# samuel-watson/glmmrMCML

Measured on AMD Instinct MI355X. Metric: MCML iters/sec x m chains (simlik evals/sec), higher is better.
Workload: dtype f64

## Files before the change

### glmmrmcml_amd/csrc/debug_hooks.hip

```cpp
#include "dgemm_mfma.h"
#include "dgemm_dl.h"
#include "dgemm_band.h"

using namespace mcml;

extern "C" int glmmr_mcml_dbg_dgemm(int M, int N, int K, const double* A, int lda,
                                    const double* B, int ldb, int b_nmajor,
                                    double alpha, double beta, double* C, int ldc,
                                    int lower_only, int force_tile)
{
    int ndev = 0;
    if (hipGetDeviceCount(&ndev) != hipSuccess || ndev == 0) {
        set_error("no HIP device: libglmmr_mcml_hip has no CPU fallback");
        return MCML_ENODEVICE;
    }
    hipStream_t s = nullptr;
    DevMat dA, dB, dC;
    if (force_tile == 40) {
        MCML_REQUIRE(!b_nmajor && !lower_only, "dbg_dgemm: the direct-to-LDS kernel takes a K-major B and all tiles");
        const int kpad = round_up(K, 32);
        MCML_TRY(dA.alloc(M, K, 32));
        MCML_HIP(hipMemset(dA.d(), 0, sizeof(double) * (size_t)dA.ld * dA.cols_alloc));
        MCML_HIP(hipMemcpy2D(dA.d(), sizeof(double) * dA.ld, A, sizeof(double) * lda, sizeof(double) * M, K, hipMemcpyHostToDevice));
        MCML_TRY(dB.alloc(kpad, N));
        MCML_HIP(hipMemset(dB.d(), 0, sizeof(double) * (size_t)dB.ld * N));
        MCML_HIP(hipMemcpy2D(dB.d(), sizeof(double) * dB.ld, B, sizeof(double) * ldb, sizeof(double) * K, N, hipMemcpyHostToDevice));
        MCML_TRY(upload_matrix(dC, C, M, N, ldc, s));
        MCML_REQUIRE(dlds_applicable(M, N, K, dA.d(), dA.ld, dA.cols_alloc, dB.d(), dB.ld), "dbg_dgemm: operands do not meet the direct-to-LDS contract");
        EpiAxpby epi2{dC.d(), dC.ld, alpha, beta};
        MCML_TRY(launch_gemm_dlds(s, M, N, K, dA.d(), dA.ld, dB.d(), dB.ld, epi2));
        MCML_TRY(download_matrix(C, ldc, dC.d(), dC.ld, M, N, s));
        return MCML_OK;
    }
    MCML_TRY(upload_matrix(dA, A, M, K, lda, s));
    if (b_nmajor) MCML_TRY(upload_matrix(dB, B, N, K, ldb, s));
    else MCML_TRY(upload_matrix(dB, B, K, N, ldb, s));
    MCML_TRY(upload_matrix(dC, C, M, N, ldc, s));
    EpiAxpby epi{dC.d(), dC.ld, alpha, beta};
    int rc;
    if (force_tile >= 20)
        rc = b_nmajor ? launch_gemm_dl<true>(s, M, N, K, dA.d(), dA.ld, dB.d(), dB.ld, epi, lower_only != 0, force_tile - 19)
                      : launch_gemm_dl<false>(s, M, N, K, dA.d(), dA.ld, dB.d(), dB.ld, epi, lower_only != 0, force_tile - 19);
    else
        rc = b_nmajor ? launch_gemm<true>(s, M, N, K, dA.d(), dA.ld, dB.d(), dB.ld, epi, lower_only != 0, force_tile)
                      : launch_gemm<false>(s, M, N, K, dA.d(), dA.ld, dB.d(), dB.ld, epi, lower_only != 0, force_tile);
    MCML_TRY(rc);
    MCML_TRY(download_matrix(C, ldc, dC.d(), dC.ld, M, N, s));
    return MCML_OK;
}

extern "C" int glmmr_mcml_dbg_dgemm_bench2(int M, int N, int K, int b_nmajor, int iters, int force_tile,
                                           int lower_only, double beta, double* ms_per_launch);
extern "C" int glmmr_mcml_dbg_dgemm_bench(int M, int N, int K, int b_nmajor, int iters,
                                          int force_tile, double* ms_per_launch)
{
    return glmmr_mcml_dbg_dgemm_bench2(M, N, K, b_nmajor, iters, force_tile, 0, 0.0, ms_per_launch);
}

extern "C" int glmmr_mcml_dbg_dgemm_bench2(int M, int N, int K, int b_nmajor, int iters, int force_tile,
                                           int lower_only, double beta, double* ms_per_launch)
{
    int ndev = 0;
    if (hipGetDeviceCount(&ndev) != hipSuccess || ndev == 0) {
        set_error("no HIP device: libglmmr_mcml_hip has no CPU fallback");
        return MCML_ENODEVICE;
    }
    hipStream_t s = nullptr;
    std::vector<double> hA((size_t)M * K), hB((size_t)K * N), hC((size_t)M * N, 0.0);
    uint64_t x = 88172645463325252ULL;
    auto rnd = [&]() { x ^= x << 13; x ^= x >> 7; x ^= x << 17; return (double)(x >> 11) / 9007199254740992.0 * 2 - 1; };
    for (auto& v : hA) v = rnd();
    for (auto& v : hB) v = rnd();
    DevMat dA, dB, dC;
    MCML_TRY(upload_matrix(dA, hA.data(), M, K, M, s));
    if (b_nmajor) MCML_TRY(upload_matrix(dB, hB.data(), N, K, N, s));
    else MCML_TRY(upload_matrix(dB, hB.data(), K, N, K, s));
    MCML_TRY(upload_matrix(dC, hC.data(), M, N, M, s));
    EpiAxpby epi{dC.d(), dC.ld, beta != 0.0 ? 1e-3 : 1.0, beta};
    const bool lo = lower_only != 0;
    auto go = [&]() {
        if (force_tile >= 20)
            return b_nmajor ? launch_gemm_dl<true>(s, M, N, K, dA.d(), dA.ld, dB.d(), dB.ld, epi, lo, force_tile - 19)
                            : launch_gemm_dl<false>(s, M, N, K, dA.d(), dA.ld, dB.d(), dB.ld, epi, lo, force_tile - 19);
        return b_nmajor ? launch_gemm<true>(s, M, N, K, dA.d(), dA.ld, dB.d(), dB.ld, epi, lo, force_tile)
                        : launch_gemm<false>(s, M, N, K, dA.d(), dA.ld, dB.d(), dB.ld, epi, lo, force_tile);
    };
    for (int i = 0; i < 3; i++) MCML_TRY(go());
    hipEvent_t e0, e1;
    MCML_HIP(hipEventCreate(&e0));
    MCML_HIP(hipEventCreate(&e1));
    MCML_HIP(hipEventRecord(e0, s));
    for (int i = 0; i < iters; i++) MCML_TRY(go());
    MCML_HIP(hipEventRecord(e1, s));
    MCML_HIP(hipEventSynchronize(e1));
    float ms = 0;
    MCML_HIP(hipEventElapsedTime(&ms, e0, e1));
    *ms_per_launch = ms / iters;
    (void)hipEventDestroy(e0);
    (void)hipEventDestroy(e1);
    return MCML_OK;
}

extern "C" int glmmr_mcml_dbg_dgemm_band(int M, int N, int K, const double* A, int lda, const double* B, int ldb,
                                         double* C, int ldc, int* tiles_executed)
{
    int ndev = 0;
    if (hipGetDeviceCount(&ndev) != hipSuccess || ndev == 0) {
        set_error("no HIP device: libglmmr_mcml_hip has no CPU fallback");
        return MCML_ENODEVICE;
    }
    MCML_REQUIRE(M > 0 && N > 0 && K > 0 && A && B && C, "dbg_dgemm_band: bad argument");
    hipStream_t s = nullptr;
    DevMat dA, dB, dC;
    MCML_TRY(dA.alloc(M, K, 32));
    MCML_HIP(hipMemset(dA.d(), 0, sizeof(double) * (size_t)dA.ld * dA.cols_alloc));
    MCML_HIP(hipMemcpy2D(dA.d(), sizeof(double) * dA.ld, A, sizeof(double) * lda, sizeof(double) * M, K, hipMemcpyHostToDevice));
    MCML_TRY(dB.alloc(round_up(K, 32), N));
    MCML_HIP(hipMemset(dB.d(), 0, sizeof(double) * (size_t)dB.ld * N));
    MCML_HIP(hipMemcpy2D(dB.d(), sizeof(double) * dB.ld, B, sizeof(double) * ldb, sizeof(double) * K, N, hipMemcpyHostToDevice));
    MCML_TRY(dC.alloc(M, N));
    MCML_HIP(hipMemset(dC.d(), 0, sizeof(double) * (size_t)dC.ld * N));
    MCML_REQUIRE(dlds_applicable(M, N, K, dA.d(), dA.ld, dA.cols_alloc, dB.d(), dB.ld), "dbg_dgemm_band: contract");
    const int nbands = (M + BD_BM - 1) / BD_BM;
    DevBuf kr;
    MCML_TRY(kr.ensure(sizeof(int) * 2 * nbands));
    hipLaunchKernelGGL(k_band_ranges, dim3(nbands), dim3(256), 0, s, dA.d(), dA.ld, M, K, kr.as<int>());
    MCML_HIP(hipGetLastError());
    std::vector<int> hk(2 * nbands);
    MCML_HIP(hipMemcpy(hk.data(), kr.p, sizeof(int) * 2 * nbands, hipMemcpyDeviceToHost));
    BandPlan plan;
    plan.reset(M, K, hk);
    if (tiles_executed) *tiles_executed = (int)plan.tiles;
    EpiAxpby epi{dC.d(), dC.ld, 1.0, 0.0};
    MCML_TRY(launch_gemm_band(s, plan, N, dA.d(), dA.ld, dB.d(), dB.ld, epi));
    MCML_TRY(download_matrix(C, ldc, dC.d(), dC.ld, M, N, s));
    return MCML_OK;
}

extern "C" int glmmr_mcml_dbg_band_clocks(int M, int N, int iters, int mode, double* out3)
{
    int ndev = 0;
    if (hipGetDeviceCount(&ndev) != hipSuccess || ndev == 0) {
        set_error("no HIP device: libglmmr_mcml_hip has no CPU fallback");
        return MCML_ENODEVICE;
    }
    hipStream_t s = nullptr;
    if (getenv("GLMMR_MCML_DBG_STREAM")) MCML_HIP(hipStreamCreateWithFlags(&s, hipStreamNonBlocking));
    std::vector<double> hA((size_t)M * M, 0.0), hB((size_t)M * N);
    uint64_t x = 88172645463325252ULL;
    auto rnd = [&]() { x ^= x << 13; x ^= x >> 7; x ^= x << 17; return (double)(x >> 11) / 9007199254740992.0 * 2 - 1; };
    const bool cst = getenv("GLMMR_MCML_DBG_DATA") && !strcmp(getenv("GLMMR_MCML_DBG_DATA"), "const");
    const bool dec = getenv("GLMMR_MCML_DBG_DATA") && !strcmp(getenv("GLMMR_MCML_DBG_DATA"), "decay");
    for (int j = 0; j < M; ++j) for (int i = j; i < M; ++i) hA[i + (size_t)j * M] = cst ? 1.0 : dec ? rnd() * std::exp(-(double)(i - j) / 40.0) : rnd();
    for (auto& v : hB) v = cst ? 1.0 : rnd();
    DevMat dA, dB, dC;
    MCML_TRY(dA.alloc(M, M, 32));
    MCML_HIP(hipMemset(dA.d(), 0, sizeof(double) * (size_t)dA.ld * dA.cols_alloc));
    MCML_HIP(hipMemcpy2D(dA.d(), sizeof(double) * dA.ld, hA.data(), sizeof(double) * M, sizeof(double) * M, M, hipMemcpyHostToDevice));
    MCML_TRY(dB.alloc(round_up(M, 32), N));
    MCML_HIP(hipMemset(dB.d(), 0, sizeof(double) * (size_t)dB.ld * N));
    MCML_HIP(hipMemcpy2D(dB.d(), sizeof(double) * dB.ld, hB.data(), sizeof(double) * M, sizeof(double) * M, N, hipMemcpyHostToDevice));
    MCML_TRY(dC.alloc(M, N));
    const int nbands = (M + BD_BM - 1) / BD_BM;
    DevBuf kr, clk;
    MCML_TRY(kr.ensure(sizeof(int) * 2 * nbands));
    MCML_TRY(clk.ensure(16));
    MCML_HIP(hipMemset(clk.p, 0, 16));
    hipLaunchKernelGGL(k_band_ranges, dim3(nbands), dim3(256), 0, s, dA.d(), dA.ld, M, M, kr.as<int>());
    std::vector<int> hk(2 * nbands);
    MCML_HIP(hipMemcpy(hk.data(), kr.p, sizeof(int) * 2 * nbands, hipMemcpyDeviceToHost));
    BandPlan plan;
    plan.reset(M, M, hk);
    const double tiles = (double)plan.tiles;
    EpiAxpby epi{dC.d(), dC.ld, 1.0, 0.0};
    if (mode < 0) {
        for (int i = 0; i < 3; i++)
            MCML_TRY((launch_gemm_band<EpiAxpby, false>(s, plan, N, dA.d(), dA.ld, dB.d(), dB.ld, epi)));
        hipEvent_t f0, f1;
        MCML_HIP(hipEventCreate(&f0));
        MCML_HIP(hipEventCreate(&f1));
        MCML_HIP(hipEventRecord(f0, s));
        for (int i = 0; i < iters; i++)
            MCML_TRY((launch_gemm_band<EpiAxpby, false>(s, plan, N, dA.d(), dA.ld, dB.d(), dB.ld, epi)));
        MCML_HIP(hipEventRecord(f1, s));
        MCML_HIP(hipEventSynchronize(f1));
        float fms = 0;
        MCML_HIP(hipEventElapsedTime(&fms, f0, f1));
        out3[0] = fms / iters; out3[1] = 0;
        out3[2] = 2.0 * 80.0 * 32.0 * tiles * N / (fms / iters * 1e-3) / 1e12;
        (void)hipEventDestroy(f0);
        (void)hipEventDestroy(f1);
        return MCML_OK;
    }
    if (mode & 16) {
        BandPlanDev* d = nullptr;
        MCML_TRY(plan.device_plan((N + BD_BN - 1) / BD_BN, s, &d));
        const int nb = d->nwg * d->gn;
        DevBuf st;
        MCML_TRY(st.ensure(sizeof(unsigned long long) * (8 + 8 * (size_t)nb)));
        for (int rep = 0; rep < 3; ++rep) {
            MCML_HIP(hipMemset(st.p, 0, sizeof(unsigned long long) * (8 + 8 * (size_t)nb)));
            MCML_TRY((launch_gemm_band<EpiAxpby, true>(s, plan, N, dA.d(), dA.ld, dB.d(), dB.ld, epi, st.as<unsigned long long>(), mode)));
            MCML_HIP(hipDeviceSynchronize());
        }
        std::vector<unsigned long long> h(8 + 8 * (size_t)nb);
        MCML_HIP(hipMemcpy(h.data(), st.p, sizeof(unsigned long long) * h.size(), hipMemcpyDeviceToHost));
        unsigned long long t0 = ~0ULL;
        for (int w = 0; w < nb; ++w) if (h[8 + 8 * w] && h[8 + 8 * w] < t0) t0 = h[8 + 8 * w];
        double mx[5] = {0, 0, 0, 0, 0}, sm[5] = {0, 0, 0, 0, 0};
        for (int w = 0; w < nb; ++w)
            for (int i = 0; i < 5; ++i) { double v = (double)(h[8 + 8 * w + i] - t0) * 0.01; sm[i] += v; if (v > mx[i]) mx[i] = v; }
        printf("band stamps (us from the first workgroup's start; %d workgroups, mean / max):\n", nb);
        const char* nm[5] = {"start", "ring filled", "K loop done", "epilogue issued", "end"};
        for (int i = 0; i < 5; ++i) printf("  %-16s %7.2f / %7.2f\n", nm[i], sm[i] / nb, mx[i]);
        if (mode & 32) for (int w = 0; w < nb; ++w) {
            printf("  wg %3d:", w);
            for (int i = 0; i < 5; ++i) printf(" %7.2f", (double)(h[8 + 8 * w + i] - t0) * 0.01);
            printf("\n");
        }
        fflush(stdout);
        out3[0] = out3[1] = out3[2] = 0;
        return MCML_OK;
    }
    for (int i = 0; i < 3; i++)
        MCML_TRY((launch_gemm_band<EpiAxpby, true>(s, plan, N, dA.d(), dA.ld, dB.d(), dB.ld, epi)));
    hipEvent_t e0, e1;
    MCML_HIP(hipEventCreate(&e0));
    MCML_HIP(hipEventCreate(&e1));
    MCML_HIP(hipEventRecord(e0, s));
    for (int i = 0; i < iters; i++)
        MCML_TRY((launch_gemm_band<EpiAxpby, true>(s, plan, N, dA.d(), dA.ld, dB.d(), dB.ld, epi, clk.as<unsigned long long>(), mode)));
    MCML_HIP(hipEventRecord(e1, s));
    MCML_HIP(hipEventSynchronize(e1));
    float ms = 0;
    MCML_HIP(hipEventElapsedTime(&ms, e0, e1));
    unsigned long long hc[2] = {0, 0};
    MCML_HIP(hipMemcpy(hc, clk.p, 16, hipMemcpyDeviceToHost));
    out3[0] = ms / iters;
    out3[1] = hc[1] ? (double)hc[0] / (double)hc[1] * 100.0 : 0.0;
    out3[2] = 2.0 * 80.0 * 32.0 * tiles * N / (ms / iters * 1e-3) / 1e12;
    (void)hipEventDestroy(e0);
    (void)hipEventDestroy(e1);
    return MCML_OK;
}

extern "C" const char* glmmr_mcml_last_error(void) { return mcml::last_error(); }

#include "rng.h"
__global__ void k_dbg_normals(uint64_t seed, uint32_t chain, uint32_t prop, uint32_t tag, int n, double* out)
{
    int i = blockIdx.x * blockDim.x + threadIdx.x;
    if (i < n) out[i] = rng_normal(seed, (uint32_t)i, chain, prop, tag);
}
__global__ void k_dbg_minstd(uint32_t seed, int n, double* out)
{
    if (threadIdx.x || blockIdx.x) return;
    uint32_t x = seed % 2147483647u;
    if (x == 0) x = 1;
    for (int i = 0; i < n; ++i) out[i] = minstd_canonical(x);
}
extern "C" int glmmr_mcml_dbg_normals(uint64_t seed, uint32_t chain, uint32_t prop, uint32_t tag, int n,
                                      double* out)
{
    DevBuf b;
    MCML_TRY(b.ensure(sizeof(double) * (size_t)n));
    hipLaunchKernelGGL(k_dbg_normals, dim3((n + 255) / 256), dim3(256), 0, nullptr, seed, chain, prop, tag, n, b.d());
    MCML_HIP(hipGetLastError());
    MCML_HIP(hipMemcpy(out, b.p, sizeof(double) * (size_t)n, hipMemcpyDeviceToHost));
    return MCML_OK;
}
extern "C" int glmmr_mcml_dbg_minstd(uint32_t seed, int n, double* out)
{
    DevBuf b;
    MCML_TRY(b.ensure(sizeof(double) * (size_t)n));
    hipLaunchKernelGGL(k_dbg_minstd, dim3(1), dim3(64), 0, nullptr, seed, n, b.d());
    MCML_HIP(hipGetLastError());
    MCML_HIP(hipMemcpy(out, b.p, sizeof(double) * (size_t)n, hipMemcpyDeviceToHost));
    return MCML_OK;
}

#include "../../include/glmmr_mcml_c.h"
#include "optim.h"
#include <cmath>
extern "C" int glmmr_mcml_dbg_bobyqa(glmmr_mcml_objective f, void* user, int n, const double* x0,
                                     const double* lower, const double* upper, double rhobeg, double rhoend,
                                     int maxfun, double* x_out, double* f_out, int* nfev_out)
{
    MCML_REQUIRE(f && n > 0 && x0 && x_out, "dbg_bobyqa: bad argument");
    objective_fn obj = [&](const std::vector<double>& x, double* v) { *v = f(x.data(), n, user); return 0; };
    std::vector<double> x(x0, x0 + n), lo(n, -HUGE_VAL), up(n, HUGE_VAL);
    if (lower) lo.assign(lower, lower + n);
    if (upper) up.assign(upper, upper + n);
    BobyqaOpts o; o.rhobeg = rhobeg; o.rhoend = rhoend; if (maxfun > 0) o.maxfun = maxfun;
    BobyqaResult r;
    MCML_TRY(bobyqa(obj, x, lo, up, o, &r));
    for (int i = 0; i < n; ++i) x_out[i] = r.x[i];
    if (f_out) *f_out = r.fval;
    if (nfev_out) *nfev_out = r.nfev;
    return MCML_OK;
}
extern "C" int glmmr_mcml_dbg_bobyqa_batch(glmmr_mcml_objective f, void* user, int n, const double* x0,
                                           const double* lower, const double* upper, double rhobeg, double rhoend,
                                           int maxfun, int width, double* x_out, double* f_out, int* nfev_out,
                                           int* rounds_out)
{
    MCML_REQUIRE(f && n > 0 && x0 && x_out && width >= 1, "dbg_bobyqa_batch: bad argument");
    batch_objective_fn obj = [&](const std::vector<std::vector<double>>& X, std::vector<double>* F) {
        F->resize(X.size());
        for (size_t i = 0; i < X.size(); ++i) (*F)[i] = f(X[i].data(), n, user);
        return 0; };
    std::vector<double> x(x0, x0 + n), lo(n, -HUGE_VAL), up(n, HUGE_VAL);
    if (lower) lo.assign(lower, lower + n);
    if (upper) up.assign(upper, upper + n);
    BobyqaOpts o; o.rhobeg = rhobeg; o.rhoend = rhoend; if (maxfun > 0) o.maxfun = maxfun;
    BobyqaResult r;
    MCML_TRY(bobyqa_batch(obj, x, lo, up, o, width, &r));
    for (int i = 0; i < n; ++i) x_out[i] = r.x[i];
    if (f_out) *f_out = r.fval;
    if (nfev_out) *nfev_out = r.nfev;
    if (rounds_out) *rounds_out = r.rounds;
    return MCML_OK;
}
extern "C" int glmmr_mcml_dbg_bobyqa_rounds(glmmr_mcml_batch_objective fb, void* user, int n, const double* x0,
                                            const double* lower, const double* upper, double rhobeg, double rhoend,
                                            int maxfun, int width, double* x_out, double* f_out, int* nfev_out,
                                            int* rounds_out)
{
    MCML_REQUIRE(fb && n > 0 && x0 && x_out && width >= 1, "dbg_bobyqa_rounds: bad argument");
    batch_objective_fn obj = [&](const std::vector<std::vector<double>>& X, std::vector<double>* F) {
        const int k = (int)X.size();
        std::vector<double> flat((size_t)n * k);
        for (int j = 0; j < k; ++j) for (int i = 0; i < n; ++i) flat[(size_t)j * n + i] = X[j][i];
        F->assign(k, 0.0);
        return fb(flat.data(), n, k, F->data(), user); };
    std::vector<double> x(x0, x0 + n), lo(n, -HUGE_VAL), up(n, HUGE_VAL);
    if (lower) lo.assign(lower, lower + n);
    if (upper) up.assign(upper, upper + n);
    BobyqaOpts o; o.rhobeg = rhobeg; o.rhoend = rhoend; if (maxfun > 0) o.maxfun = maxfun;
    BobyqaResult r;
    MCML_TRY(bobyqa_batch(obj, x, lo, up, o, width, &r));
    for (int i = 0; i < n; ++i) x_out[i] = r.x[i];
    if (f_out) *f_out = r.fval;
    if (nfev_out) *nfev_out = r.nfev;
    if (rounds_out) *rounds_out = r.rounds;
    return MCML_OK;
}
extern "C" int glmmr_mcml_dbg_fd_hessian(glmmr_mcml_objective f, void* user, int n, const double* x, double ndeps,
                                         int usebounds, const double* lower, const double* upper, double* H)
{
    MCML_REQUIRE(f && n > 0 && x && H, "dbg_fd_hessian: bad argument");
    objective_fn obj = [&](const std::vector<double>& xx, double* v) { *v = f(xx.data(), n, user); return 0; };
    std::vector<double> xv(x, x + n), nd(n, ndeps), lo(n, -HUGE_VAL), up(n, HUGE_VAL), h;
    if (lower) lo.assign(lower, lower + n);
    if (upper) up.assign(upper, upper + n);
    MCML_TRY(fd_hessian(obj, xv, nd, usebounds != 0, lo, up, &h));
    for (int i = 0; i < n * n; ++i) H[i] = h[i];
    return MCML_OK;
}

extern "C" int glmmr_mcml_dbg_copy_roundtrip(const double* in, long long ld_in, double* out, long long ld_out, long long rows, long long cols)
{
    MCML_REQUIRE(in && out && rows > 0 && cols > 0 && ld_in >= rows && ld_out >= rows, "copy_roundtrip: bad arguments");
    const size_t ldd = (size_t)rows + 3;
    DevBuf buf;
    MCML_TRY(buf.ensure(sizeof(double) * ldd * (size_t)cols));
    MCML_HIP(hipMemset(buf.p, 0xff, sizeof(double) * ldd * (size_t)cols));
    MCML_TRY(copy_h2d_2d(buf.p, sizeof(double) * ldd, in, sizeof(double) * (size_t)ld_in, sizeof(double) * (size_t)rows, (size_t)cols, 0));
    MCML_TRY(copy_d2h_2d(out, sizeof(double) * (size_t)ld_out, buf.p, sizeof(double) * ldd, sizeof(double) * (size_t)rows, (size_t)cols, 0));
    MCML_HIP(hipDeviceSynchronize());
    return MCML_OK;
}
```

### glmmrmcml_amd/csrc/dgemm_dl.h

```cpp
#pragma once
#include "dgemm_dlds.h"

namespace mcml {

template <int WTM, int WTN, int WM, int WN, bool BNMAJOR, int STAGES>
struct DlgCfg {
    static constexpr int BK = 16;
    static constexpr int NW = WM * WN, THREADS = 64 * NW;
    static constexpr int BM = 16 * WTM * WM, BN = 16 * WTN * WN;
    static constexpr int A_BYTES = BK * BM * 8, B_BYTES = BK * BN * 8;
    static constexpr int A_CHUNKS = A_BYTES / 1024, B_CHUNKS = B_BYTES / 1024;
    static constexpr int CHUNKS = A_CHUNKS + B_CHUNKS;
    static constexpr int PER = (CHUNKS + NW - 1) / NW;
    static constexpr int STAGE_BYTES = A_BYTES + B_BYTES;
    static constexpr size_t LDS_BYTES = (size_t)STAGES * STAGE_BYTES;
    static constexpr bool SWZ_A = (BM % 32) == 0;
    static constexpr bool SWZ_B = BNMAJOR && (BN % 32) == 0;
    static_assert(BM % 8 == 0 && BN % 8 == 0, "tile sides are multiples of 8 doubles");
    static_assert(LDS_BYTES <= 160 * 1024, "LDS ring does not fit");
    static_assert(PER * (STAGES - 1) <= 24, "vmcnt immediates in dl_wait_vm");
};

template <int N>
__device__ __forceinline__ void dl_wait_vm()
{
#define MCML_VM(n) else if constexpr (N == n) asm volatile("s_waitcnt vmcnt(" #n ")" ::: "memory");
    if constexpr (N <= 0) asm volatile("s_waitcnt vmcnt(0)" ::: "memory");
    MCML_VM(1) MCML_VM(2) MCML_VM(3) MCML_VM(4) MCML_VM(5) MCML_VM(6) MCML_VM(7) MCML_VM(8)
    MCML_VM(9) MCML_VM(10) MCML_VM(11) MCML_VM(12) MCML_VM(13) MCML_VM(14) MCML_VM(15) MCML_VM(16)
    MCML_VM(17) MCML_VM(18) MCML_VM(19) MCML_VM(20) MCML_VM(21) MCML_VM(22) MCML_VM(23) MCML_VM(24)
    else asm volatile("s_waitcnt vmcnt(0)" ::: "memory");
#undef MCML_VM
}

template <int PER, int MAXT>
__device__ __forceinline__ void dl_wait_leave(int tiles)
{
    if constexpr (MAXT <= 0) dl_wait_vm<0>();
    else {
        if (tiles >= MAXT) dl_wait_vm<PER * MAXT>();
        else dl_wait_leave<PER, MAXT - 1>(tiles);
    }
}

template <int WTM, int WTN, int WM, int WN, bool BNMAJOR, int STAGES, class Epi>
__global__ __launch_bounds__(64 * WM * WN) void dgemm_dl_kernel(GemmP p, Epi epi)
{
    using Cfg = DlgCfg<WTM, WTN, WM, WN, BNMAJOR, STAGES>;
    constexpr int BM = Cfg::BM, BN = Cfg::BN, BK = Cfg::BK, NW = Cfg::NW, PER = Cfg::PER;
    extern __shared__ __attribute__((aligned(16))) double smem[];
    char* lds = reinterpret_cast<char*>(smem);
    const int tid = threadIdx.x, lane = tid & 63, wave = __builtin_amdgcn_readfirstlane(tid >> 6);
    const int wr = wave / WN, wc = wave - wr * WN;

    const int nblk = gridDim.x;
    const int bid = blockIdx.x;
    const int q8 = nblk >> 3, r8 = nblk & 7, xcd = bid & 7;
    const int nid = (xcd < r8 ? xcd * (q8 + 1) : r8 * (q8 + 1) + (xcd - r8) * q8) + (bid >> 3);
    int bi, bj;
    if (p.lower_only) {
        int rem = nid;
        for (bi = 0; bi < p.gm; ++bi) {
            int nc = (bi * BM + BM - 1 + p.diag_shift) / BN + 1;
            if (nc > p.gn) nc = p.gn;
            if (rem < nc) break;
            rem -= nc;
        }
        bj = rem;
    } else {
        bi = nid / p.gn; bj = nid - bi * p.gn;
    }
    const int m0 = bi * BM, n0 = bj * BN;

    unsigned voff[PER]; int loff[PER]; bool isA[PER];
#pragma unroll
    for (int s = 0; s < PER; ++s) {
        int c = wave + NW * s;
        if (c >= Cfg::CHUNKS) c = wave;
        isA[s] = c < Cfg::A_CHUNKS;
        if (c < Cfg::A_CHUNKS) {
            const int o = c * 1024 + lane * 16;
            const int k = o / (BM * 8), pos = (o - k * BM * 8) >> 3;
            const int m = Cfg::SWZ_A ? ((((pos >> 4) ^ (k & 1)) << 4) | (pos & 15)) : pos;
            int gm = m0 + m;
            if (gm >= p.M) gm = 0;
            voff[s] = (unsigned)((gm + (size_t)k * p.lda) * 8);
            loff[s] = c * 1024;
        } else {
            const int cb = c - Cfg::A_CHUNKS;
            const int o = cb * 1024 + lane * 16;
            if (BNMAJOR) {
                const int k = o / (BN * 8), pos = (o - k * BN * 8) >> 3;
                const int n = Cfg::SWZ_B ? ((((pos >> 4) ^ (k & 1)) << 4) | (pos & 15)) : pos;
                int gn = n0 + n;
                if (gn >= p.N) gn = 0;
                voff[s] = (unsigned)((gn + (size_t)k * p.ldb) * 8);
            } else {
                const int q = o >> 4;
                const int kp = q / BN, n = q - kp * BN;
                int gn = n0 + n;
                if (gn >= p.N) gn = 0;
                voff[s] = (unsigned)((2 * kp + (size_t)gn * p.ldb) * 8);
            }
            loff[s] = Cfg::A_BYTES + cb * 1024;
        }
    }
    const size_t stepA = (size_t)BK * p.lda * 8, stepB = BNMAJOR ? (size_t)BK * p.ldb * 8 : (size_t)BK * 8;
    const int by = blockIdx.y;
    const char* sA = reinterpret_cast<const char*>(p.A + (size_t)by * p.bsA);
    const char* sB = reinterpret_cast<const char*>(p.B + (size_t)by * p.bsB);

    auto issue = [&](int stage) {
        const unsigned lbase = (unsigned)(size_t)(lds_ptr_t)lds + stage * Cfg::STAGE_BYTES;
#pragma unroll
        for (int s = 0; s < PER; ++s) lds_dma16(lbase + loff[s], voff[s], isA[s] ? sA : sB);
        sA += stepA;
        sB += stepB;
    };

    d4 acc[WTM][WTN];
#pragma unroll
    for (int i = 0; i < WTM; ++i)
#pragma unroll
        for (int j = 0; j < WTN; ++j) acc[i][j] = d4{0.0, 0.0, 0.0, 0.0};

    const int l15 = lane & 15, lk = lane >> 4;
    auto compute = [&](int stage) {
        const double* as = reinterpret_cast<const double*>(lds + stage * Cfg::STAGE_BYTES);
        const double* bs = reinterpret_cast<const double*>(lds + stage * Cfg::STAGE_BYTES + Cfg::A_BYTES);
#pragma unroll
        for (int ks = 0; ks < BK / 4; ++ks) {
            const int kk = 4 * ks + lk;
            double a[WTM], b[WTN];
#pragma unroll
            for (int i = 0; i < WTM; ++i) {
                const int blk = wr * WTM + i;
                a[i] = as[kk * BM + ((Cfg::SWZ_A ? (blk ^ (kk & 1)) : blk) << 4) + l15];
            }
#pragma unroll
            for (int j = 0; j < WTN; ++j) {
                const int blk = wc * WTN + j;
                if (BNMAJOR) b[j] = bs[kk * BN + ((Cfg::SWZ_B ? (blk ^ (kk & 1)) : blk) << 4) + l15];
                else b[j] = bs[((kk >> 1) * BN + (blk << 4) + l15) * 2 + (kk & 1)];
            }
#pragma unroll
            for (int i = 0; i < WTM; ++i)
#pragma unroll
                for (int j = 0; j < WTN; ++j)
                    acc[i][j] = __builtin_amdgcn_mfma_f64_16x16x4f64(b[j], a[i], acc[i][j], 0, 0, 0);
        }
    };

    const int nk = p.K / BK;
    int issued = 0;
    for (; issued < STAGES - 1 && issued < nk; ++issued) issue(issued);
    dl_wait_leave<PER, STAGES - 2>(issued - 1);
    __builtin_amdgcn_s_barrier();
    int st = 0;
    for (int kt = 0; kt < nk; ++kt) {
        if (issued < nk) {
            int sn = st + STAGES - 1; if (sn >= STAGES) sn -= STAGES;
            issue(sn);
            ++issued;
        }
        compute(st);
        dl_wait_leave<PER, STAGES - 2>(issued - kt - 2);
        __builtin_amdgcn_s_barrier();
        st = st + 1; if (st >= STAGES) st = 0;
    }

    Epi e = epi;
    e.shift(by);
    e(acc, m0 + wr * 16 * WTM, n0 + wc * 16 * WTN, lane, p.M, p.N, bi * WM + wr);
}

static inline bool dl_applicable(int M, int N, int K, const double* A, int lda, const double* B, int ldb,
                                 bool bnmajor)
{
    return M >= 1 && N >= 1 && K >= 16 && (K & 15) == 0 && ((uintptr_t)A & 15) == 0 && ((uintptr_t)B & 15) == 0 &&
           (lda & 1) == 0 && (ldb & 1) == 0 && lda >= M && (bnmajor ? ldb >= N : ldb >= K) &&
           dma_offsets_fit((size_t)lda * 16 + M, bnmajor ? (size_t)ldb * 16 + N : (size_t)ldb * N + 16);
}

template <int WTM, int WTN, int WM, int WN, bool BNMAJOR, int STAGES, class Epi>
static inline int launch_gemm_dl_cfg(hipStream_t s, GemmP p, const Epi& epi, int nbatch = 1)
{
    using Cfg = DlgCfg<WTM, WTN, WM, WN, BNMAJOR, STAGES>;
    p.gm = (p.M + Cfg::BM - 1) / Cfg::BM;
    p.gn = (p.N + Cfg::BN - 1) / Cfg::BN;
    long ntiles = (long)p.gm * p.gn;
    if (p.lower_only) {
        ntiles = 0;
        for (int bi = 0; bi < p.gm; ++bi) {
            int nc = (bi * Cfg::BM + Cfg::BM - 1 + p.diag_shift) / Cfg::BN + 1;
            ntiles += nc > p.gn ? p.gn : nc;
        }
    }
    MCML_TRY(ensure_dynamic_lds(reinterpret_cast<const void*>(&dgemm_dl_kernel<WTM, WTN, WM, WN, BNMAJOR, STAGES, Epi>), (int)Cfg::LDS_BYTES));
    hipLaunchKernelGGL((dgemm_dl_kernel<WTM, WTN, WM, WN, BNMAJOR, STAGES, Epi>), dim3((unsigned)ntiles, (unsigned)nbatch),
                       dim3(Cfg::THREADS), Cfg::LDS_BYTES, s, p, epi);
    MCML_HIP(hipGetLastError());
    return MCML_OK;
}

template <bool BNMAJOR, class Epi>
static inline int launch_gemm_dl(hipStream_t s, int M, int N, int K, const double* A, int lda,
                                 const double* B, int ldb, const Epi& epi, bool lower_only = false, int tile = 0,
                                 int inplace = 0, int diag_shift = 0, int nbatch = 1, size_t bsA = 0, size_t bsB = 0)
{
    MCML_REQUIRE(dl_applicable(M, N, K, A, lda, B, ldb, BNMAJOR), "dgemm_dl: shape/alignment contract violated "
                 "(M %d N %d K %d lda %d ldb %d)", M, N, K, lda, ldb);
    GemmP p{M, N, K, A, lda, B, ldb, 0, 0, lower_only ? 1 : 0, 0, diag_shift, bsA, bsB};
    if (tile == 0) {
        long t128 = (long)((M + 127) / 128) * ((N + 127) / 128);
        if (lower_only) t128 = t128 / 2 + (M + 127) / 128;
        static const int big = getenv("GLMMR_MCML_DL_BIG") ? atoi(getenv("GLMMR_MCML_DL_BIG")) : 4;
        static const int small = getenv("GLMMR_MCML_DL_SMALL") ? atoi(getenv("GLMMR_MCML_DL_SMALL")) : 5;
        static const int thr = getenv("GLMMR_MCML_DL_THR") ? atoi(getenv("GLMMR_MCML_DL_THR")) : 768;
        static const int thr64 = getenv("GLMMR_MCML_DL_THR64") ? atoi(getenv("GLMMR_MCML_DL_THR64")) : 128;
        tile = t128 >= thr ? big : small;
        if (inplace == 0 && t128 < thr64) tile = 6;
        if (inplace == 2) tile = N >= 256 ? 3 : 1;
    }
    MCML_REQUIRE(!(inplace == 1 && (tile == 6 || tile == 8) && N > (tile == 6 ? 64 : 32)) &&
                 !(inplace == 2 && (tile == 2 || tile == 5 || tile == 6 || tile == 7 || tile == 8) && M > (tile == 7 ? 16 : tile == 8 ? 32 : 64)),
                 "dgemm_dl: tile %d cannot run this product in place", tile);
    if (tile == 1) return launch_gemm_dl_cfg<4, 2, 2, 4, BNMAJOR, 4, Epi>(s, p, epi, nbatch);
    if (tile == 3) return launch_gemm_dl_cfg<1, 2, 8, 1, BNMAJOR, 6, Epi>(s, p, epi, nbatch);
    if (tile == 4) return launch_gemm_dl_cfg<4, 2, 2, 4, BNMAJOR, 2, Epi>(s, p, epi, nbatch);
    if (tile == 5) return launch_gemm_dl_cfg<2, 2, 2, 4, BNMAJOR, 3, Epi>(s, p, epi, nbatch);
    if (tile == 6) return launch_gemm_dl_cfg<2, 2, 2, 2, BNMAJOR, 3, Epi>(s, p, epi, nbatch);
    if (tile == 7) return launch_gemm_dl_cfg<1, 2, 1, 4, BNMAJOR, 4, Epi>(s, p, epi, nbatch);
    if (tile == 8) return launch_gemm_dl_cfg<1, 1, 2, 2, BNMAJOR, 4, Epi>(s, p, epi, nbatch);
    return launch_gemm_dl_cfg<2, 2, 2, 4, BNMAJOR, 5, Epi>(s, p, epi, nbatch);
}

}
```

### include/glmmr_mcml_c.h

```cpp
#ifndef GLMMR_MCML_C_H
#define GLMMR_MCML_C_H
#include <stdint.h>

#ifdef __cplusplus
extern "C" {
#endif

#define GLMMR_MCML_OK            0
#define GLMMR_MCML_EINVAL       -1
#define GLMMR_MCML_EUNSUPPORTED -2
#define GLMMR_MCML_ENOTPD       -3
#define GLMMR_MCML_ESINGULAR    -4
#define GLMMR_MCML_EHIP         -5
#define GLMMR_MCML_ENODEVICE    -6
#define GLMMR_MCML_ENOMEM       -7

const char* glmmr_mcml_last_error(void);


typedef struct glmmr_mcml_problem {
    const int32_t* cov;
    int            cov_rows;
    const double*  data;
    int            data_len;
    const double*  eff_range;
    int            eff_len;
    const double*  Z;
    const double*  X;
    const double*  y;
    int            n, Q, P;
    const char*    family;
    const char*    link;
} glmmr_mcml_problem;

typedef int (*glmmr_mcml_reduce_fn)(void* user, double* dev_buf, int n);

typedef struct glmmr_mcml_dev_opts {
    int   device;
    void* stream;
    int   rank, world;
    glmmr_mcml_reduce_fn reduce;
    void* reduce_user;
} glmmr_mcml_dev_opts;

typedef struct glmmr_mcml_ctx glmmr_mcml_ctx;

int glmmr_mcml_ctx_create(const glmmr_mcml_problem* prob, const glmmr_mcml_dev_opts* opts,
                          glmmr_mcml_ctx** out);
int glmmr_mcml_ctx_destroy(glmmr_mcml_ctx* ctx);

#define GLMMR_MCML_RCCL_ID_BYTES 128
int glmmr_mcml_rccl_unique_id(unsigned char* id128);
int glmmr_mcml_ctx_comm_init_rccl(glmmr_mcml_ctx* ctx, const unsigned char* id128, int rank, int world);
int glmmr_mcml_ctx_comm_allreduce(glmmr_mcml_ctx* ctx, double* vals, int n);

int glmmr_mcml_ctx_comm_stats(glmmr_mcml_ctx* ctx, long long* calls, long long* doubles, int* native);
int glmmr_mcml_ctx_shard_stats(glmmr_mcml_ctx* ctx, long long* out6);

int glmmr_mcml_set_u(glmmr_mcml_ctx* ctx, const double* u, int Q, int ncols, int niter);
int glmmr_mcml_get_u(glmmr_mcml_ctx* ctx, double* u, int ldu);
int glmmr_mcml_get_u_all(glmmr_mcml_ctx* ctx, double* u, int ldu, int* ncols_out);

int glmmr_mcml_ctx_mvn_ll(glmmr_mcml_ctx* ctx, const double* theta, double* out);
int glmmr_mcml_ctx_mvn_ll_batch(glmmr_mcml_ctx* ctx, const double* thetas, int k, double* out);
int glmmr_mcml_ctx_gen_D(glmmr_mcml_ctx* ctx, const double* theta, int chol, double* out, int ldo);

int glmmr_mcml_ctx_loglik(glmmr_mcml_ctx* ctx, const double* beta, double var_par, double* out);
int glmmr_mcml_ctx_mcnr(glmmr_mcml_ctx* ctx, const double* beta, double var_par, double* beta_out,
                        double* sigma_out, double* stats_out);
int glmmr_mcml_ctx_update_L(glmmr_mcml_ctx* ctx, const double* theta);
int glmmr_mcml_ctx_set_L(glmmr_mcml_ctx* ctx, const double* L, int ldl);

typedef struct glmmr_mcml_hmc_opts {
    int    warmup;
    int    nsamp;
    int    adapt;
    double lambda;
    int    max_steps;
    double target_accept;
    int    chains;
    int    chain_offset;
} glmmr_mcml_hmc_opts;

typedef struct glmmr_mcml_hmc_diag {
    double    accept_rate, mean_e, min_e, max_e;
    int       max_steps_used;
    long long leapfrog_total;
} glmmr_mcml_hmc_diag;

int glmmr_mcml_ctx_hmc_sample(glmmr_mcml_ctx* ctx, const double* beta, double var_par,
                              const glmmr_mcml_hmc_opts* opts, uint64_t seed, uint32_t iter_idx,
                              const double* inj_init, const double* inj_mom, uint8_t* flags_out,
                              double* probs_out, glmmr_mcml_hmc_diag* diag, int* ncols_out);

typedef struct glmmr_mcml_nuts_opts {
    int    warmup;
    int    nsamp;
    int    max_treedepth;
    double adapt_delta;
    double stepsize;
    int    chains;
    int    chain_offset;
    int    metric;
} glmmr_mcml_nuts_opts;

typedef struct glmmr_mcml_nuts_diag {
    double    mean_e, min_e, max_e;
    long long divergent;
    long long treedepth_hits;
    long long batched_leapfrogs;
    long long stepsize_search_leapfrogs;
} glmmr_mcml_nuts_diag;

int glmmr_mcml_ctx_nuts_sample(glmmr_mcml_ctx* ctx, const double* beta, double var_par,
                               const glmmr_mcml_nuts_opts* opts, uint64_t seed, uint32_t iter_idx,
                               int* depth_out, int* nleap_out, double* eps_out, double* accept_out,
                               glmmr_mcml_nuts_diag* diag, int* ncols_out);


typedef struct glmmr_mcml_ext {
    uint64_t seed;
    int      chains;
    int      maxfun;
    int      device;
    int      theta_batch;
} glmmr_mcml_ext;

int glmmr_mcml_gen_u_samples(const double* Z, const double* L, const double* X, const double* y, int n, int Q, int P,
                             const double* beta, const char* family, const char* link, double sigma, int warmup_iter,
                             int m, const glmmr_mcml_nuts_opts* opts, const glmmr_mcml_ext* ext, double* samples,
                             int lds, int* ncols);

int glmmr_mcml_sample_cols(int m, int chains);
int glmmr_mcml_ctx_ncols(glmmr_mcml_ctx* ctx);
int glmmr_mcml_ctx_profile(glmmr_mcml_ctx* ctx, int enable, int reset, double* out8);
int glmmr_mcml_ctx_profile_launches(glmmr_mcml_ctx* ctx, long long* fwd, long long* bwd);
int glmmr_mcml_ctx_last_kernels(glmmr_mcml_ctx* ctx, int* fwd, int* bwd);
int glmmr_mcml_dbg_band_plan(glmmr_mcml_ctx* ctx, int which, int chains, int* out10);
int glmmr_mcml_dbg_phase_ms(int enable, int reset, double* out8);
int glmmr_mcml_ctx_npar(glmmr_mcml_ctx* ctx);

int glmmr_mcml_ctx_optim(glmmr_mcml_ctx* ctx, const double* start, int nstart, int trace, int mcnr,
                         const glmmr_mcml_ext* ext, double* beta, double* theta, double* sigma);
int glmmr_mcml_ctx_simlik(glmmr_mcml_ctx* ctx, const double* start, int nstart, int trace,
                          const glmmr_mcml_ext* ext, double* beta, double* theta, double* sigma);
int glmmr_mcml_ctx_hess(glmmr_mcml_ctx* ctx, const double* start, int nstart, double tol, int trace,
                        double* H );
int glmmr_mcml_ctx_aic(glmmr_mcml_ctx* ctx, const double* beta_par, int nbeta, const double* cov_par,
                       int ncov, double* out);
int glmmr_mcml_ctx_full(glmmr_mcml_ctx* ctx, const double* start, int nstart, int mcnr, int m, int maxiter,
                        int warmup, double tol, int verbose, double lambda, int trace, int refresh,
                        int maxsteps, double target_accept, const glmmr_mcml_ext* ext, double* beta,
                        double* theta, double* sigma, int* converged, int* iters,
                        glmmr_mcml_hmc_diag* last_diag);

int glmmr_mcml_full(const glmmr_mcml_problem* prob, const double* start, int nstart, int mcnr, int m,
                    int maxiter, int warmup, double tol, int verbose, double lambda, int trace,
                    int refresh, int maxsteps, double target_accept, const glmmr_mcml_ext* ext,
                    double* beta, double* theta, double* sigma, int* converged, double* u, int ldu,
                    int* ucols);

int glmmr_mcml_mcmc_sample(const double* Z, const double* L, const double* X, const double* y, int n,
                           int Q, int P, const double* beta, const char* family, const char* link,
                           int warmup, int nsamp, double lambda, double var_par, int trace, int refresh,
                           int maxsteps, double target_accept, const glmmr_mcml_ext* ext,
                           double* samples, int lds, int* ncols);

int glmmr_mcml_optim(const glmmr_mcml_problem* prob, const double* u, int ucols, const double* start,
                     int nstart, int trace, int mcnr, const glmmr_mcml_ext* ext, double* beta,
                     double* theta, double* sigma);
int glmmr_mcml_simlik(const glmmr_mcml_problem* prob, const double* u, int ucols, const double* start,
                      int nstart, int trace, const glmmr_mcml_ext* ext, double* beta, double* theta,
                      double* sigma);
int glmmr_mcml_optim_sparse(const glmmr_mcml_problem* prob, const int32_t* Ap, const int32_t* Ai, int nnz,
                            const double* u, int ucols, const double* start, int nstart, int trace,
                            int mcnr, const glmmr_mcml_ext* ext, double* beta, double* theta,
                            double* sigma,
                            int32_t* Lp, int32_t* Li, double* Lx, double* D, int lcap);
int glmmr_mcml_sparse_factor_nnz(const int32_t* cov, int cov_rows, const double* data, int data_len);
int glmmr_mcml_simlik_sparse(const glmmr_mcml_problem* prob, const int32_t* Ap, const int32_t* Ai, int nnz,
                             const double* u, int ucols, const double* start, int nstart, int trace,
                             const glmmr_mcml_ext* ext, double* beta, double* theta, double* sigma);
int glmmr_mcml_hess(const glmmr_mcml_problem* prob, const double* u, int ucols, const double* start,
                    int nstart, double tol, int trace, const glmmr_mcml_ext* ext, double* H);
int glmmr_mcml_hess_sparse(const glmmr_mcml_problem* prob, const int32_t* Ap, const int32_t* Ai, int nnz,
                           const double* u, int ucols, const double* start, int nstart, double tol,
                           int trace, const glmmr_mcml_ext* ext, double* H);
int glmmr_mcml_aic(const glmmr_mcml_problem* prob, const double* u, int ucols, const double* beta_par,
                   int nbeta, const double* cov_par, int ncov, const glmmr_mcml_ext* ext, double* out);

int glmmr_mcml_la(const glmmr_mcml_problem* prob, const double* start, int nstart, int usehess, double tol,
                  int verbose, int trace, int maxiter, const glmmr_mcml_ext* ext, double* beta, double* theta,
                  double* sigma, double* se, double* u);
int glmmr_mcml_la_nr(const glmmr_mcml_problem* prob, const double* start, int nstart, int usehess, double tol,
                     int verbose, int trace, int maxiter, const glmmr_mcml_ext* ext, double* beta, double* theta,
                     double* sigma, double* se, double* u);
int glmmr_mcml_ctx_la(glmmr_mcml_ctx* ctx, const double* start, int nstart, int nr, int usehess, double tol,
                      int verbose, int trace, int maxiter, const glmmr_mcml_ext* ext, double* beta, double* theta,
                      double* sigma, double* se, double* u, int* converged, int* iters);

int glmmr_mcml_mvn_ll(const int32_t* cov, int cov_rows, const double* data, int data_len,
                      const double* eff_range, int eff_len, const double* gamma, int ngamma,
                      const double* u, int Q, int m, double* out);

int glmmr_mcml_dbg_theta_log(glmmr_mcml_ctx* ctx, int enable, double* out, int cap_rows, int* nrows);
int glmmr_mcml_dbg_emulate_world(glmmr_mcml_ctx* ctx, int world, int mode);
int glmmr_mcml_dbg_leaf_profile(glmmr_mcml_ctx* ctx, unsigned long long* out10);
int glmmr_mcml_dbg_la_probe(glmmr_mcml_ctx* ctx, const double* start, int nstart, int kind, const double* v,
                            double var_par, const double* par, int npar, double* out, double* v_out,
                            double* beta_out, double* sigma_out);
int glmmr_mcml_dbg_dgemm(int M, int N, int K, const double* A, int lda, const double* B, int ldb,
                         int b_nmajor, double alpha, double beta, double* C, int ldc,
                         int lower_only, int force_tile );
int glmmr_mcml_dbg_log_prob_grad(glmmr_mcml_ctx* ctx, const double* beta, double var_par, const double* V,
                                 int ncols, double* lp, double* G);
int glmmr_mcml_dbg_normals(uint64_t seed, uint32_t chain, uint32_t prop, uint32_t tag, int n, double* out);
int glmmr_mcml_dbg_minstd(uint32_t seed, int n, double* out);
typedef double (*glmmr_mcml_objective)(const double* x, int n, void* user);
int glmmr_mcml_dbg_bobyqa(glmmr_mcml_objective f, void* user, int n, const double* x0, const double* lower,
                          const double* upper, double rhobeg, double rhoend, int maxfun, double* x_out,
                          double* f_out, int* nfev_out);
int glmmr_mcml_dbg_bobyqa_batch(glmmr_mcml_objective f, void* user, int n, const double* x0, const double* lower,
                                const double* upper, double rhobeg, double rhoend, int maxfun, int width,
                                double* x_out, double* f_out, int* nfev_out, int* rounds_out);
typedef int (*glmmr_mcml_batch_objective)(const double* X, int n, int k, double* F, void* user);
int glmmr_mcml_dbg_bobyqa_rounds(glmmr_mcml_batch_objective fb, void* user, int n, const double* x0, const double* lower,
                                 const double* upper, double rhobeg, double rhoend, int maxfun, int width,
                                 double* x_out, double* f_out, int* nfev_out, int* rounds_out);
int glmmr_mcml_dbg_copy_roundtrip(const double* in, long long ld_in, double* out, long long ld_out, long long rows, long long cols);
int glmmr_mcml_dbg_fd_hessian(glmmr_mcml_objective f, void* user, int n, const double* x, double ndeps,
                              int usebounds, const double* lower, const double* upper, double* H);
int glmmr_mcml_dbg_dgemm_bench(int M, int N, int K, int b_nmajor, int iters, int force_tile,
                               double* ms_per_launch);
int glmmr_mcml_dbg_dgemm_bench2(int M, int N, int K, int b_nmajor, int iters, int force_tile, int lower_only,
                                double beta, double* ms_per_launch);
int glmmr_mcml_dbg_dgemm_band(int M, int N, int K, const double* A, int lda, const double* B, int ldb, double* C,
                              int ldc, int* tiles_executed);
int glmmr_mcml_dbg_band_clocks(int M, int N, int iters, int mode, double* out3);

#ifdef __cplusplus
}
#endif
#endif
```

Before: 1116.

## Software-pipeline LDS fragment reads against MFMA in direct-to-LDS DGEMM inner loop

Replaces the K-step compute loop of the direct-to-LDS DGEMM kernel with a double-buffered register pipeline. Hand-issued ds_read_b64 loads for the next sub-step run while MFMAs consume the current fragments, gated by explicit lgkmcnt waits and sched_barriers. The next stage's first fragments are prefetched right after the barrier. The aim is to hide LDS read latency behind matrix-core work. The old loop is kept behind a template flag and a new debug entry point, and the inline asm plus manual waitcnt accounting risks ordering bugs or extra register pressure.

New measurement: 1120, median of 6. Within noise of the previous version (+0.3%).

```diff
diff --git a/glmmrmcml_amd/csrc/debug_hooks.hip b/glmmrmcml_amd/csrc/debug_hooks.hip
--- a/glmmrmcml_amd/csrc/debug_hooks.hip
+++ b/glmmrmcml_amd/csrc/debug_hooks.hip
@@ -46,6 +46,57 @@
                       : launch_gemm<false>(s, M, N, K, dA.d(), dA.ld, dB.d(), dB.ld, epi, lower_only != 0, force_tile);
     MCML_TRY(rc);
     MCML_TRY(download_matrix(C, ldc, dC.d(), dC.ld, M, N, s));
+    return MCML_OK;
+}
+
+extern "C" int glmmr_mcml_dbg_dgemm_dl(int M, int N, int K, double* A, int lda, long long lenA, double* B, int ldb,
+                                       long long lenB, int b_nmajor, double alpha, double beta, double* C, int ldc,
+                                       long long lenC, int lower_only, int tile, int inplace, int diag_shift,
+                                       int nbatch, long long bsA, long long bsB, long long bsC, int old_loop)
+{
+    int ndev = 0;
+    if (hipGetDeviceCount(&ndev) != hipSuccess || ndev == 0) {
+        set_error("no HIP device: libglmmr_mcml_hip has no CPU fallback");
+        return MCML_ENODEVICE;
+    }
+    MCML_REQUIRE(M > 0 && N > 0 && K > 0 && A && B && nbatch >= 1 && tile >= 1 && tile <= 8 && inplace >= 0 && inplace <= 2 &&
+                 (inplace != 0 || C), "dbg_dgemm_dl: bad argument");
+    if (inplace == 1) { ldc = lda; bsC = bsA; }
+    if (inplace == 2) { ldc = ldb; bsC = bsB; }
+    const long long last = nbatch - 1;
+    MCML_REQUIRE(last * bsA + (long long)lda * (K - 1) + M <= lenA &&
+                 last * bsB + (b_nmajor ? (long long)ldb * (K - 1) + N : (long long)ldb * (N - 1) + K) <= lenB &&
+                 last * bsC + (long long)ldc * (N - 1) + M <= (inplace == 1 ? lenA : inplace == 2 ? lenB : lenC) &&
+                 ldc >= M, "dbg_dgemm_dl: operands do not fit their buffers");
+    hipStream_t s = nullptr;
+    DevBuf dA, dB, dC;
+    MCML_TRY(dA.ensure(sizeof(double) * (size_t)lenA));
+    MCML_TRY(dB.ensure(sizeof(double) * (size_t)lenB));
+    MCML_TRY(copy_h2d(dA.p, A, sizeof(double) * (size_t)lenA, s));
+    MCML_TRY(copy_h2d(dB.p, B, sizeof(double) * (size_t)lenB, s));
+    double* Cd = inplace == 1 ? dA.as<double>() : inplace == 2 ? dB.as<double>() : nullptr;
+    if (inplace == 0) {
+        MCML_TRY(dC.ensure(sizeof(double) * (size_t)lenC));
+        MCML_TRY(copy_h2d(dC.p, C, sizeof(double) * (size_t)lenC, s));
+        Cd = dC.as<double>();
+    }
+    EpiAxpby epi{Cd, ldc, alpha, beta, (size_t)bsC};
+    const bool lo = lower_only != 0;
+    const double* Ad = dA.as<double>();
+    const double* Bd = dB.as<double>();
+    int rc;
+    if (b_nmajor)
+        rc = old_loop ? launch_gemm_dl<true, EpiAxpby, true>(s, M, N, K, Ad, lda, Bd, ldb, epi, lo, tile, inplace, diag_shift, nbatch, bsA, bsB)
+                      : launch_gemm_dl<true, EpiAxpby, false>(s, M, N, K, Ad, lda, Bd, ldb, epi, lo, tile, inplace, diag_shift, nbatch, bsA, bsB);
+    else
+        rc = old_loop ? launch_gemm_dl<false, EpiAxpby, true>(s, M, N, K, Ad, lda, Bd, ldb, epi, lo, tile, inplace, diag_shift, nbatch, bsA, bsB)
+                      : launch_gemm_dl<false, EpiAxpby, false>(s, M, N, K, Ad, lda, Bd, ldb, epi, lo, tile, inplace, diag_shift, nbatch, bsA, bsB);
+    MCML_TRY(rc);
+    double* hout = inplace == 1 ? A : inplace == 2 ? B : C;
+    const DevBuf& dout = inplace == 1 ? dA : inplace == 2 ? dB : dC;
+    const long long lenout = inplace == 1 ? lenA : inplace == 2 ? lenB : lenC;
+    MCML_TRY(copy_d2h(hout, dout.p, sizeof(double) * (size_t)lenout, s));
+    MCML_HIP(hipStreamSynchronize(s));
     return MCML_OK;
 }
 
diff --git a/glmmrmcml_amd/csrc/dgemm_dl.h b/glmmrmcml_amd/csrc/dgemm_dl.h
--- a/glmmrmcml_amd/csrc/dgemm_dl.h
+++ b/glmmrmcml_amd/csrc/dgemm_dl.h
@@ -43,7 +43,47 @@
     }
 }
 
-template <int WTM, int WTN, int WM, int WN, bool BNMAJOR, int STAGES, class Epi>
+#if defined(__HIP_DEVICE_COMPILE__)
+#define DL_RD(dst, addr, off) asm volatile("ds_read_b64 %0, %1 offset:%2" : "=v"(dst) : "v"(addr), "i"(off))
+#else
+#define DL_RD(dst, addr, off) (dst = 0.0)
+#endif
+template <int KS, int BM, int BN, int WTM, int WTN>
+__device__ __forceinline__ void dl_read(double (&a)[WTM], double (&b)[WTN], const unsigned (&aaddr)[WTM],
+                                        const unsigned (&baddr)[WTN])
+{
+#pragma unroll
+    for (int i = 0; i < WTM; ++i) DL_RD(a[i], aaddr[i], KS * 4 * BM * 8);
+#pragma unroll
+    for (int j = 0; j < WTN; ++j) DL_RD(b[j], baddr[j], KS * 4 * BN * 8);
+}
+template <int N, int WTM, int WTN>
+__device__ __forceinline__ void dl_wait_lgkm(double (&a)[WTM], double (&b)[WTN])
+{
+#if defined(__HIP_DEVICE_COMPILE__)
+    static_assert(N >= 0 && N <= 8, "lgkmcnt immediates below");
+#define MCML_LG(n) else if constexpr (N == n) asm volatile("s_waitcnt lgkmcnt(" #n ")" ::: "memory");
+    if constexpr (N == 0) asm volatile("s_waitcnt lgkmcnt(0)" ::: "memory");
+    MCML_LG(1) MCML_LG(2) MCML_LG(3) MCML_LG(4) MCML_LG(5) MCML_LG(6) MCML_LG(7) MCML_LG(8)
+#undef MCML_LG
+#pragma unroll
+    for (int i = 0; i < WTM; ++i) asm volatile("" : "+v"(a[i]));
+#pragma unroll
+    for (int j = 0; j < WTN; ++j) asm volatile("" : "+v"(b[j]));
+#else
+    (void)a; (void)b;
+#endif
+}
+template <int WTM, int WTN>
+__device__ __forceinline__ void dl_mfma(d4 (&acc)[WTM][WTN], const double (&a)[WTM], const double (&b)[WTN])
+{
+#pragma unroll
+    for (int i = 0; i < WTM; ++i)
+#pragma unroll
+        for (int j = 0; j < WTN; ++j) acc[i][j] = __builtin_amdgcn_mfma_f64_16x16x4f64(b[j], a[i], acc[i][j], 0, 0, 0);
+}
+
+template <int WTM, int WTN, int WM, int WN, bool BNMAJOR, int STAGES, class Epi, bool OLDK = false>
 __global__ __launch_bounds__(64 * WM * WN) void dgemm_dl_kernel(GemmP p, Epi epi)
 {
     using Cfg = DlgCfg<WTM, WTN, WM, WN, BNMAJOR, STAGES>;
@@ -157,16 +197,67 @@
     dl_wait_leave<PER, STAGES - 2>(issued - 1);
     __builtin_amdgcn_s_barrier();
     int st = 0;
-    for (int kt = 0; kt < nk; ++kt) {
-        if (issued < nk) {
-            int sn = st + STAGES - 1; if (sn >= STAGES) sn -= STAGES;
-            issue(sn);
-            ++issued;
-        }
-        compute(st);
-        dl_wait_leave<PER, STAGES - 2>(issued - kt - 2);
-        __builtin_amdgcn_s_barrier();
-        st = st + 1; if (st >= STAGES) st = 0;
+    if constexpr (OLDK) {
+        for (int kt = 0; kt < nk; ++kt) {
+            if (issued < nk) {
+                int sn = st + STAGES - 1; if (sn >= STAGES) sn -= STAGES;
+                issue(sn);
+                ++issued;
+            }
+            compute(st);
+            dl_wait_leave<PER, STAGES - 2>(issued - kt - 2);
+            __builtin_amdgcn_s_barrier();
+            st = st + 1; if (st >= STAGES) st = 0;
+        }
+    } else {
+        static_assert(BK == 16, "four substeps per K step below");
+        constexpr int RD = WTM + WTN;
+        const unsigned lds0 = (unsigned)(size_t)(lds_ptr_t)lds;
+        unsigned a0[WTM], b0[WTN], aa[WTM], ba[WTN];
+#pragma unroll
+        for (int i = 0; i < WTM; ++i) {
+            const int blk = wr * WTM + i;
+            a0[i] = lds0 + 8 * (lk * BM + ((Cfg::SWZ_A ? (blk ^ (lk & 1)) : blk) << 4) + l15);
+        }
+#pragma unroll
+        for (int j = 0; j < WTN; ++j) {
+            const int blk = wc * WTN + j;
+            if (BNMAJOR) b0[j] = lds0 + Cfg::A_BYTES + 8 * (lk * BN + ((Cfg::SWZ_B ? (blk ^ (lk & 1)) : blk) << 4) + l15);
+            else b0[j] = lds0 + Cfg::A_BYTES + 8 * ((((lk >> 1) * BN + (blk << 4) + l15) << 1) + (lk & 1));
+        }
+        auto at_stage = [&](int s) {
+#pragma unroll
+            for (int i = 0; i < WTM; ++i) aa[i] = a0[i] + s * Cfg::STAGE_BYTES;
+#pragma unroll
+            for (int j = 0; j < WTN; ++j) ba[j] = b0[j] + s * Cfg::STAGE_BYTES;
+        };
+        double ra[2][WTM], rb[2][WTN];
+        at_stage(0);
+        dl_read<0, BM, BN>(ra[0], rb[0], aa, ba);
+        for (int kt = 0; kt < nk; ++kt) {
+            if (issued < nk) {
+                int sn = st + STAGES - 1; if (sn >= STAGES) sn -= STAGES;
+                issue(sn);
+                ++issued;
+            }
+#define DL_STEP(KS, CUR, NXT)                                  \
+            dl_read<KS + 1, BM, BN>(ra[NXT], rb[NXT], aa, ba); \
+            dl_wait_lgkm<RD>(ra[CUR], rb[CUR]);                \
+            dl_mfma(acc, ra[CUR], rb[CUR]);                    \
+            __builtin_amdgcn_sched_barrier(0);
+            DL_STEP(0, 0, 1) DL_STEP(1, 1, 0) DL_STEP(2, 0, 1)
+#undef DL_STEP
+            dl_wait_leave<PER, STAGES - 2>(issued - kt - 2);
+            dl_wait_lgkm<0>(ra[1], rb[1]);
+            __builtin_amdgcn_s_barrier();
+            st = st + 1; if (st >= STAGES) st = 0;
+            if (kt + 1 < nk) {
+                at_stage(st);
+                dl_read<0, BM, BN>(ra[0], rb[0], aa, ba);
+            }
+            dl_mfma(acc, ra[1], rb[1]);
+            __builtin_amdgcn_sched_barrier(0);
+        }
     }
 
     Epi e = epi;
@@ -182,7 +273,7 @@
            dma_offsets_fit((size_t)lda * 16 + M, bnmajor ? (size_t)ldb * 16 + N : (size_t)ldb * N + 16);
 }
 
-template <int WTM, int WTN, int WM, int WN, bool BNMAJOR, int STAGES, class Epi>
+template <int WTM, int WTN, int WM, int WN, bool BNMAJOR, int STAGES, class Epi, bool OLDK = false>
 static inline int launch_gemm_dl_cfg(hipStream_t s, GemmP p, const Epi& epi, int nbatch = 1)
 {
     using Cfg = DlgCfg<WTM, WTN, WM, WN, BNMAJOR, STAGES>;
@@ -196,14 +287,14 @@
             ntiles += nc > p.gn ? p.gn : nc;
         }
     }
-    MCML_TRY(ensure_dynamic_lds(reinterpret_cast<const void*>(&dgemm_dl_kernel<WTM, WTN, WM, WN, BNMAJOR, STAGES, Epi>), (int)Cfg::LDS_BYTES));
-    hipLaunchKernelGGL((dgemm_dl_kernel<WTM, WTN, WM, WN, BNMAJOR, STAGES, Epi>), dim3((unsigned)ntiles, (unsigned)nbatch),
+    MCML_TRY(ensure_dynamic_lds(reinterpret_cast<const void*>(&dgemm_dl_kernel<WTM, WTN, WM, WN, BNMAJOR, STAGES, Epi, OLDK>), (int)Cfg::LDS_BYTES));
+    hipLaunchKernelGGL((dgemm_dl_kernel<WTM, WTN, WM, WN, BNMAJOR, STAGES, Epi, OLDK>), dim3((unsigned)ntiles, (unsigned)nbatch),
                        dim3(Cfg::THREADS), Cfg::LDS_BYTES, s, p, epi);
     MCML_HIP(hipGetLastError());
     return MCML_OK;
 }
 
-template <bool BNMAJOR, class Epi>
+template <bool BNMAJOR, class Epi, bool OLDK = false>
 static inline int launch_gemm_dl(hipStream_t s, int M, int N, int K, const double* A, int lda,
                                  const double* B, int ldb, const Epi& epi, bool lower_only = false, int tile = 0,
                                  int inplace = 0, int diag_shift = 0, int nbatch = 1, size_t bsA = 0, size_t bsB = 0)
@@ -225,14 +316,14 @@
     MCML_REQUIRE(!(inplace == 1 && (tile == 6 || tile == 8) && N > (tile == 6 ? 64 : 32)) &&
                  !(inplace == 2 && (tile == 2 || tile == 5 || tile == 6 || tile == 7 || tile == 8) && M > (tile == 7 ? 16 : tile == 8 ? 32 : 64)),
                  "dgemm_dl: tile %d cannot run this product in place", tile);
-    if (tile == 1) return launch_gemm_dl_cfg<4, 2, 2, 4, BNMAJOR, 4, Epi>(s, p, epi, nbatch);
-    if (tile == 3) return launch_gemm_dl_cfg<1, 2, 8, 1, BNMAJOR, 6, Epi>(s, p, epi, nbatch);
-    if (tile == 4) return launch_gemm_dl_cfg<4, 2, 2, 4, BNMAJOR, 2, Epi>(s, p, epi, nbatch);
-    if (tile == 5) return launch_gemm_dl_cfg<2, 2, 2, 4, BNMAJOR, 3, Epi>(s, p, epi, nbatch);
-    if (tile == 6) return launch_gemm_dl_cfg<2, 2, 2, 2, BNMAJOR, 3, Epi>(s, p, epi, nbatch);
-    if (tile == 7) return launch_gemm_dl_cfg<1, 2, 1, 4, BNMAJOR, 4, Epi>(s, p, epi, nbatch);
-    if (tile == 8) return launch_gemm_dl_cfg<1, 1, 2, 2, BNMAJOR, 4, Epi>(s, p, epi, nbatch);
-    return launch_gemm_dl_cfg<2, 2, 2, 4, BNMAJOR, 5, Epi>(s, p, epi, nbatch);
-}
-
-}
+    if (tile == 1) return launch_gemm_dl_cfg<4, 2, 2, 4, BNMAJOR, 4, Epi, OLDK>(s, p, epi, nbatch);
+    if (tile == 3) return launch_gemm_dl_cfg<1, 2, 8, 1, BNMAJOR, 6, Epi, OLDK>(s, p, epi, nbatch);
+    if (tile == 4) return launch_gemm_dl_cfg<4, 2, 2, 4, BNMAJOR, 2, Epi, OLDK>(s, p, epi, nbatch);
+    if (tile == 5) return launch_gemm_dl_cfg<2, 2, 2, 4, BNMAJOR, 3, Epi, OLDK>(s, p, epi, nbatch);
+    if (tile == 6) return launch_gemm_dl_cfg<2, 2, 2, 2, BNMAJOR, 3, Epi, OLDK>(s, p, epi, nbatch);
+    if (tile == 7) return launch_gemm_dl_cfg<1, 2, 1, 4, BNMAJOR, 4, Epi, OLDK>(s, p, epi, nbatch);
+    if (tile == 8) return launch_gemm_dl_cfg<1, 1, 2, 2, BNMAJOR, 4, Epi, OLDK>(s, p, epi, nbatch);
+    return launch_gemm_dl_cfg<2, 2, 2, 4, BNMAJOR, 5, Epi, OLDK>(s, p, epi, nbatch);
+}
+
+}
diff --git a/include/glmmr_mcml_c.h b/include/glmmr_mcml_c.h
--- a/include/glmmr_mcml_c.h
+++ b/include/glmmr_mcml_c.h
@@ -212,6 +212,10 @@
 int glmmr_mcml_dbg_dgemm(int M, int N, int K, const double* A, int lda, const double* B, int ldb,
                          int b_nmajor, double alpha, double beta, double* C, int ldc,
                          int lower_only, int force_tile );
+int glmmr_mcml_dbg_dgemm_dl(int M, int N, int K, double* A, int lda, long long lenA, double* B, int ldb,
+                            long long lenB, int b_nmajor, double alpha, double beta, double* C, int ldc,
+                            long long lenC, int lower_only, int tile, int inplace, int diag_shift,
+                            int nbatch, long long bsA, long long bsB, long long bsC, int old_loop);
 int glmmr_mcml_dbg_log_prob_grad(glmmr_mcml_ctx* ctx, const double* beta, double var_par, const double* V,
                                  int ncols, double* lp, double* G);
 int glmmr_mcml_dbg_normals(uint64_t seed, uint32_t chain, uint32_t prop, uint32_t tag, int n, double* out);
```
